# avianphysics/avian

Hardware: NVIDIA H100
Metric: physics steps/sec on 100k-cube stack (broad phase + solver stage per step) (higher is better)
Workload: dtype f32

## Files before the change

avian_b200/csrc/contact_rows.hpp:

```cpp
#pragma once
#include <cstdint>

#include "narrow_math.hpp"

namespace avn {

template <class S>
struct EdgeRows {
    int E;
    uint32_t* c1; uint32_t* c2; uint32_t* b1; uint32_t* b2; uint8_t* live;
    uint8_t* count; uint8_t* disjoint; S* normal; S* a1; S* a2; S* pen; S* ns;
    uint8_t* prev_count; double* prev_a1; double* prev_a2;
    S* ws_n_in; S* ws_t_in; S* ws_n_out; S* ws_t_out; S* nimp_in; S* nimp_out;
};

template <class S>
struct NarrowEdgeArgs {
    EdgeRows<S> r;
    const uint8_t* shape; const S* dims; const S* pos; const S* rot; const S* lv; const S* av; const S* amin; const S* amax;
    double dt, tol, thr2;
    int match;
};

template <class S> NM_HD inline nm::V3 ldd3(const S* p, size_t i) { return {double(p[3 * i]), double(p[3 * i + 1]), double(p[3 * i + 2])}; }
template <class S> NM_HD inline void std3(S* p, size_t i, nm::V3 v) { p[3 * i] = S(v.x); p[3 * i + 1] = S(v.y); p[3 * i + 2] = S(v.z); }

template <class S>
NM_HD inline void narrow_edge_row(const NarrowEdgeArgs<S>& a, int e) {
    const EdgeRows<S>& r = a.r;
    if (!r.live[e]) { r.count[e] = 0; r.disjoint[e] = 0; return; }
    const uint32_t ca = r.c1[e], cb = r.c2[e], ba = r.b1[e], bb = r.b2[e];
    int np = 0;
    nm::V3 normal{0, 0, 0};
    nm::PointOut out[4];
    bool disjoint = false;
    {
        const nm::V3 mina = ldd3(a.amin, ca), maxa = ldd3(a.amax, ca), minb = ldd3(a.amin, cb), maxb = ldd3(a.amax, cb);
        disjoint = (mina.x > maxb.x || maxa.x < minb.x || mina.y > maxb.y || maxa.y < minb.y || mina.z > maxb.z || maxa.z < minb.z);
    }
    r.disjoint[e] = disjoint ? 1 : 0;
    if (!disjoint) {
        const nm::V3 pa = ldd3(a.pos, ca), pb = ldd3(a.pos, cb);
        const nm::Q qa{double(a.rot[4 * size_t(ca)]), double(a.rot[4 * size_t(ca) + 1]), double(a.rot[4 * size_t(ca) + 2]), double(a.rot[4 * size_t(ca) + 3])};
        const nm::Q qb{double(a.rot[4 * size_t(cb)]), double(a.rot[4 * size_t(cb) + 1]), double(a.rot[4 * size_t(cb) + 2]), double(a.rot[4 * size_t(cb) + 3])};
        const nm::V3 v1 = ldd3(a.lv, ba), v2 = ldd3(a.lv, bb), w1 = ldd3(a.av, ba), w2 = ldd3(a.av, bb);
        const nm::V3 rel = v2 - v1;
        const double eff_margin = a.dt * nm::len(rel);
        const double max_dist = nm::smax(eff_margin, a.tol);
        nm::Contacts pts;
        const int ta = a.shape ? a.shape[ca] : nm::SHAPE_CUBOID, tb = a.shape ? a.shape[cb] : nm::SHAPE_CUBOID;
        if (nm::collide(ta, ldd3(a.dims, ca), pa, qa, tb, ldd3(a.dims, cb), pb, qb, max_dist, normal, pts))
            np = nm::manifold_points(pts, normal, pa, pb, rel, w1, w2, a.dt, eff_margin, out);
        else
            normal = nm::V3{0, 0, 0};
    }
    const int oc = r.prev_count[e];
    nm::V3 oa1[4], oa2[4];
    S on[4], otx[4], oty[4];
    for (int k = 0; k < oc; ++k) {
        const size_t q = size_t(e) * 4 + k;
        oa1[k] = nm::V3{r.prev_a1[3 * q], r.prev_a1[3 * q + 1], r.prev_a1[3 * q + 2]};
        oa2[k] = nm::V3{r.prev_a2[3 * q], r.prev_a2[3 * q + 1], r.prev_a2[3 * q + 2]};
        on[k] = r.ws_n_out[q]; otx[k] = r.ws_t_out[2 * q]; oty[k] = r.ws_t_out[2 * q + 1];
    }
    r.count[e] = uint8_t(np);
    std3(r.normal, size_t(e), normal);
    for (int k = 0; k < 4; ++k) {
        const size_t q = size_t(e) * 4 + k;
        S vn = S(0), vx = S(0), vy = S(0);
        if (k < np) {
            const int j = a.match ? nm::match_point(out[k].anchor1, out[k].anchor2, oa1, oa2, oc, a.thr2) : -1;
            if (j >= 0) { vn = on[j]; vx = otx[j]; vy = oty[j]; }
            std3(r.a1, q, out[k].anchor1);
            std3(r.a2, q, out[k].anchor2);
            r.pen[q] = S(out[k].penetration);
            r.ns[q] = S(out[k].normal_speed);
            r.prev_a1[3 * q] = out[k].anchor1.x; r.prev_a1[3 * q + 1] = out[k].anchor1.y; r.prev_a1[3 * q + 2] = out[k].anchor1.z;
            r.prev_a2[3 * q] = out[k].anchor2.x; r.prev_a2[3 * q + 1] = out[k].anchor2.y; r.prev_a2[3 * q + 2] = out[k].anchor2.z;
        } else {
            std3(r.a1, q, nm::V3{0, 0, 0});
            std3(r.a2, q, nm::V3{0, 0, 0});
            r.pen[q] = S(0);
            r.ns[q] = S(0);
        }
        r.ws_n_in[q] = vn;
        r.ws_t_in[2 * q] = vx;
        r.ws_t_in[2 * q + 1] = vy;
        r.ws_n_out[q] = vn;
        r.ws_t_out[2 * q] = vx;
        r.ws_t_out[2 * q + 1] = vy;
    }
    r.prev_count[e] = uint8_t(np);
}


}
```

avian_b200/csrc/contacts.cu:

```cuda
#include <cooperative_groups.h>

#include <algorithm>
#include <cstdlib>
#include <cstring>

#include "context.hpp"
#include "contact_rows.hpp"
#include "device_prims.cuh"

namespace avn {
namespace {
namespace cg = cooperative_groups;

enum { CH_NONE = 0, CH_PUSH = 1, CH_POP = 2, CH_REMOVE = 3, CH_MASK = 3, CH_DONE = 0x10 };
enum { ISL_NONE = 0, ISL_ADD = 1, ISL_REMOVE = 2 };

struct GraphCounters {
    uint32_t removed, started, stopped, changed, rounds, ovf_dirty, manifolds, any_restitution, aborted, bad_pairs;
    uint32_t round_left[3];
    uint32_t color_offsets[AVN_GRAPH_COLOR_COUNT + 1];
    uint32_t ovf_count;
};

struct GraphRows {
// ... 268 lines not shown
}

__global__ void pair_set_kernel(GraphRows g, uint64_t* __restrict__ table, uint64_t mask) {
    const int e = blockIdx.x * blockDim.x + threadIdx.x;
    if (e >= g.hw || !g.live[e]) return;
    const uint32_t a = g.c1[e], b = g.c2[e];
    const uint64_t k = (a < b ? (uint64_t(a) << 32) | b : (uint64_t(b) << 32) | a) + 1;
    uint64_t h = hash64(k) & mask;
    for (;;) {
        unsigned long long prev = atomicCAS((unsigned long long*)&table[h], 0ull, (unsigned long long)k);
        if (prev == 0ull || prev == k) return;
        h = (h + 1) & mask;
    }
}

__global__ void edge_add_kernel(int n, const uint32_t* __restrict__ ids, const uint32_t* __restrict__ c1, const uint32_t* __restrict__ c2,
                                const uint32_t* __restrict__ b1, const uint32_t* __restrict__ b2, uint32_t* rc1, uint32_t* rc2, uint32_t* rb1, uint32_t* rb2,
                                uint8_t* live, uint8_t* count, uint8_t* prev_count) {
    int k = blockIdx.x * blockDim.x + threadIdx.x;
    if (k >= n) return;
    const uint32_t e = ids[k];
    rc1[e] = c1[k]; rc2[e] = c2[k]; rb1[e] = b1[k]; rb2[e] = b2[k];
    live[e] = 1;
    count[e] = 0;
    prev_count[e] = 0;
}
__global__ void edge_remove_kernel(int n, const uint32_t* __restrict__ ids, uint8_t* live, uint8_t* count, uint8_t* prev_count) {
    int k = blockIdx.x * blockDim.x + threadIdx.x;
    if (k >= n) return;
    const uint32_t e = ids[k];
    live[e] = 0; count[e] = 0; prev_count[e] = 0;
}

template <class S>
__global__ void __launch_bounds__(128) narrow_edges_kernel(const __grid_constant__ NarrowEdgeArgs<S> a, uint8_t* fresh, int only_fresh) {
    const int e = blockIdx.x * blockDim.x + threadIdx.x;
    if (e >= a.r.E) return;
    if (only_fresh) {
        if (!fresh[e]) return;
        fresh[e] = 0;
    }
    narrow_edge_row<S>(a, e);
}


struct IslandCounters { uint32_t islands, sleeping, put_to_sleep, woken, split_bodies, merges, split_root, _pad; unsigned long long cand; };
constexpr uint32_t ISL_NONE_BODY = 0xffffffffu;

struct IslandState {
    int B;
    const uint8_t* kind;
    uint32_t* parent; uint32_t* root; uint32_t* root_prev; uint32_t* removed;
    uint8_t* isl_sleeping; uint8_t* awake; uint8_t* need_wake; uint8_t* touched; uint8_t* in_split;
    float* timer;
    const float* thr_lin; const float* thr_ang; const uint8_t* disabled; const uint8_t* host_wake;
    uint32_t* cand_body;
    IslandCounters* ctr;
    float time_to_sleep, delta_secs;
};
__device__ __forceinline__ bool isl_static(const IslandState& s, uint32_t b) { return b >= uint32_t(s.B) || s.kind[b] == AVN_BODY_STATIC; }
__device__ __forceinline__ uint32_t isl_find(uint32_t* parent, uint32_t x) {
    uint32_t p = *reinterpret_cast<volatile uint32_t*>(&parent[x]);
    while (p != x) {
        const uint32_t gp = *reinterpret_cast<volatile uint32_t*>(&parent[p]);
        if (gp != p) parent[x] = gp;
        x = p; p = gp;
    }
    return x;
}
__device__ __forceinline__ bool isl_union(uint32_t* parent, uint32_t u, uint32_t v) {
    for (;;) {
        uint32_t ru = isl_find(parent, u), rv = isl_find(parent, v);
        if (ru == rv) return false;
        if (ru < rv) { const uint32_t t = ru; ru = rv; rv = t; }
        if (atomicCAS(&parent[ru], ru, rv) == ru) return true;
// ... 120 lines not shown
    if (b >= s.B || isl_static(s, uint32_t(b)) || s.root[b] != uint32_t(b)) return;
    atomicAdd(&s.ctr->islands, 1u);
    if (!s.awake[b] && !s.isl_sleeping[b] && s.removed[b] == 0) { s.isl_sleeping[b] = 1; atomicAdd(&s.ctr->put_to_sleep, 1u); }
    if (s.isl_sleeping[b]) atomicAdd(&s.ctr->sleeping, 1u);
}
__global__ void isl_finish_kernel(IslandState s, uint32_t* __restrict__ out_island, uint8_t* __restrict__ out_sleeping) {
    const int b = blockIdx.x * blockDim.x + threadIdx.x;
    if (b >= s.B) return;
    const bool st = isl_static(s, uint32_t(b));
    const uint32_t r = st ? ISL_NONE_BODY : s.root[b];
    out_island[b] = r;
    out_sleeping[b] = (!st && s.isl_sleeping[r]) ? 1 : 0;
    s.root_prev[b] = st ? uint32_t(b) : r;
    s.awake[b] = 0; s.need_wake[b] = 0; s.touched[b] = 0; s.in_split[b] = 0;
    if (b == 0) {
        const unsigned long long c = s.ctr->cand;
        if (c != 0ull) *s.cand_body = 0xffffffffu - uint32_t(c & 0xffffffffull);
    }
}

template <class S>
class Contacts final : public ContactsBase {
   public:
    Contacts(cudaStream_t stream, ErrorSink* err) : stream_(stream), err_(err) {
        int dev = 0;
        cudaGetDevice(&dev);
        cudaDeviceProp prop;
        if (cudaGetDeviceProperties(&prop, dev) == cudaSuccess) sm_count_ = prop.multiProcessorCount;
        cudaHostAlloc(&h_ctr_, sizeof(GraphCounters), cudaHostAllocDefault);
        up_stream_ = stream_;
        if (cudaStreamCreateWithFlags(&copy_stream_, cudaStreamNonBlocking) != cudaSuccess) { (void)cudaGetLastError(); copy_stream_ = nullptr; }
        cudaEventCreateWithFlags(&ev_in_, cudaEventDisableTiming);
        if (const char* c = getenv("AVN_GRAPH_CLUSTER")) use_cluster_ = atoi(c) != 0;
    }
    ~Contacts() override {
        if (h_ctr_) cudaFreeHost(h_ctr_);
        if (h_isl_) cudaFreeHost(h_isl_);
        if (ev_in_) cudaEventDestroy(ev_in_);
        if (copy_stream_) { cudaStreamSynchronize(copy_stream_); cudaStreamDestroy(copy_stream_); }
    }

    AvnStatus reserve(uint32_t capacity) override {
        if (capacity <= E_) return AVN_OK;
        const size_t n = capacity;
        struct Col { DevBuf* buf; size_t bytes_per_row; };
        Col cols[] = {{&c1_, 4}, {&c2_, 4}, {&b1_, 4}, {&b2_, 4}, {&live_, 1}, {&count_, 1}, {&disjoint_, 1}, {&normal_, 3 * sizeof(S)}, {&a1_, 12 * sizeof(S)},
                      {&a2_, 12 * sizeof(S)}, {&pen_, 4 * sizeof(S)}, {&ns_, 4 * sizeof(S)}, {&prev_count_, 1}, {&prev_a1_, 12 * sizeof(double)},
                      {&prev_a2_, 12 * sizeof(double)}, {&ws_n_in_, 4 * sizeof(S)}, {&ws_t_in_, 8 * sizeof(S)}, {&ws_n_out_, 4 * sizeof(S)},
                      {&ws_t_out_, 8 * sizeof(S)}, {&nimp_in_, 4 * sizeof(S)}, {&nimp_out_, 4 * sizeof(S)},
                      {&pflags_, 1}, {&touching_, 1}, {&colour_, 1}, {&change_, 1}, {&old_colour_, 1}, {&ovf_pos_, 4}, {&ovf_, 4}, {&isl_event_, 1}, {&fresh_, 1}};
        for (Col& c : cols) {
            void* fresh = nullptr;
            AVN_CUDA(cudaMalloc(&fresh, n * c.bytes_per_row));
            AVN_CUDA(cudaMemsetAsync(fresh, 0, n * c.bytes_per_row, stream_));
            if (c.buf->p && E_) AVN_CUDA(cudaMemcpyAsync(fresh, c.buf->p, size_t(E_) * c.bytes_per_row, cudaMemcpyDeviceToDevice, stream_));
            AVN_CUDA(cudaStreamSynchronize(stream_));
            if (c.buf->p) cudaFree(c.buf->p);
            c.buf->p = fresh;
            c.buf->cap = n * c.bytes_per_row;
        }
        E_ = capacity;
        const size_t nblocks = (n + RS_TILE - 1) / RS_TILE;
        AVN_CUDA(k0_.ensure(n * 4)); AVN_CUDA(k1_.ensure(n * 4)); AVN_CUDA(v0_.ensure(n * 4)); AVN_CUDA(v1_.ensure(n * 4)); AVN_CUDA(list_.ensure(n * 4));
        AVN_CUDA(hist_.ensure(256 * nblocks * 4));
        AVN_CUDA(m_b1_.ensure(n * 4)); AVN_CUDA(m_b2_.ensure(n * 4)); AVN_CUDA(m_fr_.ensure(n * sizeof(S))); AVN_CUDA(m_re_.ensure(n * sizeof(S)));
        uint64_t cap = 1024;
// ... 357 lines not shown
        UPC(i_lv_, in->linear_velocity, 3 * B, S, in_.lv);
        UPC(i_av_, in->angular_velocity, 3 * B, S, in_.av);
        UPC(i_amin_, in->aabb_min, 3 * C, S, in_.amin);
        UPC(i_amax_, in->aabb_max, 3 * C, S, in_.amax);
#undef UPC
        up_stream_ = stream_;
        in_.colliders = C;
        return AVN_OK;
    }
    AvnStatus launch_narrow(const AvnNarrowParams* prm, const AvnNarrowInput* in, uint32_t match_contacts, double length_unit, uint32_t n) {
        bool only_fresh = false;
        if (prefetched_ == in) {
            AVN_CUDA(cudaStreamWaitEvent(stream_, ev_in_, 0));
            only_fresh = early_rows_ > 0;
            if (only_fresh && n == early_rows_ && !added_this_step_) { prefetched_ = nullptr; early_rows_ = 0; return AVN_OK; }
        } else {
            if (prefetched_) AVN_CUDA(cudaStreamWaitEvent(stream_, ev_in_, 0));
            AvnStatus st = upload_inputs(in, false, stream_);
            if (st != AVN_OK) return st;
        }
        prefetched_ = nullptr;
        early_rows_ = 0;
        return enqueue_narrow(prm, match_contacts, length_unit, n, stream_, only_fresh);
    }
    AvnStatus enqueue_narrow(const AvnNarrowParams* prm, uint32_t match_contacts, double length_unit, uint32_t n, cudaStream_t s, bool only_fresh) {
        NarrowEdgeArgs<S> a{};
        a.r = rows();
        a.r.E = int(n);
        a.shape = in_.shape; a.dims = in_.dims; a.pos = in_.pos; a.rot = in_.rot; a.lv = in_.lv; a.av = in_.av; a.amin = in_.amin; a.amax = in_.amax;
        a.dt = prm->dt;
        a.tol = prm->contact_tolerance;
        a.thr2 = (0.1 * length_unit) * (0.1 * length_unit);
        a.match = match_contacts ? 1 : 0;
        narrow_edges_kernel<S><<<(n + 127) / 128, 128, 0, s>>>(a, fresh_.as<uint8_t>(), only_fresh ? 1 : 0);
        AVN_CUDA(cudaGetLastError());
        return AVN_OK;
    }
    void radix_pass(int n) {
        const int nblocks = (n + RS_TILE - 1) / RS_TILE;
        rs_histogram<uint32_t><<<nblocks, RS_THREADS, 0, stream_>>>(k0_.as<uint32_t>(), n, 0, hist_.as<uint32_t>(), nblocks);
        if (nblocks <= RS_FUSE_MAX_BLOCKS) {
            rs_scatter<uint32_t, true><<<nblocks, RS_THREADS, 0, stream_>>>(k0_.as<uint32_t>(), v0_.as<uint32_t>(), n, 0, hist_.as<uint32_t>(), nblocks, k1_.as<uint32_t>(),
                                                                            v1_.as<uint32_t>());
        } else {
            rs_scan<<<1, 1024, 0, stream_>>>(hist_.as<uint32_t>(), 256 * nblocks);
            rs_scatter<uint32_t, false><<<nblocks, RS_THREADS, 0, stream_>>>(k0_.as<uint32_t>(), v0_.as<uint32_t>(), n, 0, hist_.as<uint32_t>(), nblocks, k1_.as<uint32_t>(),
                                                                             v1_.as<uint32_t>());
        }
    }
    GraphRows graph_rows() {
        GraphRows g{};
        g.hw = int(hw_);
        g.c1 = c1_.as<uint32_t>(); g.c2 = c2_.as<uint32_t>(); g.b1 = b1_.as<uint32_t>(); g.b2 = b2_.as<uint32_t>();
        g.live = live_.as<uint8_t>(); g.count = count_.as<uint8_t>(); g.disjoint = disjoint_.as<uint8_t>(); g.prev_count = prev_count_.as<uint8_t>();
        g.pflags = pflags_.as<uint8_t>(); g.touching = touching_.as<uint8_t>(); g.colour = colour_.as<uint8_t>(); g.change = change_.as<uint8_t>();
        g.old_colour = old_colour_.as<uint8_t>(); g.ovf_pos = ovf_pos_.as<uint32_t>(); g.ovf = ovf_.as<uint32_t>(); g.isl_event = isl_event_.as<uint8_t>(); g.fresh = fresh_.as<uint8_t>();
        g.body_kind = kind_.as<uint8_t>(); g.n_bodies = int(n_bodies_);
        g.body_bits = body_bits_.as<uint32_t>(); g.body_min = body_min_.as<unsigned long long>();
        g.ctr = ctr_.as<GraphCounters>();
        return g;
    }
    EdgeRows<S> rows() {
        EdgeRows<S> r{};
        r.E = int(E_);
        r.c1 = c1_.as<uint32_t>(); r.c2 = c2_.as<uint32_t>(); r.b1 = b1_.as<uint32_t>(); r.b2 = b2_.as<uint32_t>(); r.live = live_.as<uint8_t>();
        r.count = count_.as<uint8_t>(); r.disjoint = disjoint_.as<uint8_t>(); r.normal = normal_.as<S>(); r.a1 = a1_.as<S>(); r.a2 = a2_.as<S>();
        r.pen = pen_.as<S>(); r.ns = ns_.as<S>(); r.prev_count = prev_count_.as<uint8_t>(); r.prev_a1 = prev_a1_.as<double>(); r.prev_a2 = prev_a2_.as<double>();
// ... 52 lines not shown
```

avian_b200/csrc/narrow_math.hpp:

```cpp
#pragma once
#include <cmath>

#if defined(__CUDACC__)
#define NM_HD __host__ __device__
#define NM_COLD __host__ __device__ __noinline__
#define NM_ROLLED _Pragma("unroll 1")
#else
#define NM_HD
#define NM_COLD
#define NM_ROLLED
#endif

namespace nm {

using S = double;

struct V3 { S x, y, z; };
NM_HD inline V3 operator+(V3 a, V3 b) { return {a.x + b.x, a.y + b.y, a.z + b.z}; }
NM_HD inline V3 operator-(V3 a, V3 b) { return {a.x - b.x, a.y - b.y, a.z - b.z}; }
NM_HD inline V3 operator-(V3 a) { return {-a.x, -a.y, -a.z}; }
NM_HD inline V3 operator*(V3 a, S s) { return {a.x * s, a.y * s, a.z * s}; }
NM_HD inline S dot(V3 a, V3 b) { return a.x * b.x + a.y * b.y + a.z * b.z; }
NM_HD inline V3 cross(V3 a, V3 b) { return {a.y * b.z - a.z * b.y, a.z * b.x - a.x * b.z, a.x * b.y - a.y * b.x}; }
NM_HD inline S len(V3 a) { return sqrt(dot(a, a)); }
NM_HD inline S comp(V3 a, int i) { return i == 0 ? a.x : (i == 1 ? a.y : a.z); }
NM_HD inline S smax(S a, S b) { return a < b ? b : a; }
NM_HD inline S smin(S a, S b) { return b < a ? b : a; }

struct Q { S x, y, z, w; };
NM_HD inline V3 rot(Q q, V3 v) {
    V3 b{q.x, q.y, q.z};
    S b2 = dot(b, b);
    return v * (q.w * q.w - b2) + b * (dot(v, b) * 2) + cross(b, v) * (q.w * 2);
}
struct M3 { V3 c[3]; };
NM_HD inline M3 to_mat(Q q) { return {{rot(q, {1, 0, 0}), rot(q, {0, 1, 0}), rot(q, {0, 0, 1})}}; }

enum ShapeType { SHAPE_CUBOID = 0, SHAPE_SPHERE = 1 };
struct Box { V3 c; M3 r; V3 he; };

constexpr int MAX_RAW_POINTS = 8;
struct Witness { V3 a, b; };
struct Contacts {
    int n;
    Witness p[MAX_RAW_POINTS];
    NM_HD void clear() { n = 0; }
    NM_HD void push(V3 on_a, V3 on_b) { p[n].a = on_a; p[n].b = on_b; ++n; }
};

NM_HD inline void box_face(const Box& b, int axis, S sign, V3 out[4]) {
    int u = (axis + 1) % 3, v = (axis + 2) % 3;
    V3 n = b.r.c[axis] * (sign * comp(b.he, axis));
    V3 eu = b.r.c[u] * comp(b.he, u), ev = b.r.c[v] * comp(b.he, v);
    V3 fc = b.c + n;
    out[0] = fc + eu + ev; out[1] = fc - eu + ev; out[2] = fc - eu - ev; out[3] = fc + eu - ev;
}

NM_HD inline int clip_poly(const V3* in, int n, V3 plane_n, S plane_d, V3* out) {
    int m = 0;
    for (int i = 0; i < n; ++i) {
        V3 a = in[i], b = in[(i + 1) % n];
        S da = dot(plane_n, a) - plane_d, db = dot(plane_n, b) - plane_d;
        if (da <= 0) out[m++] = a;
        if ((da < 0 && db > 0) || (da > 0 && db < 0)) out[m++] = a + (b - a) * (da / (da - db));
    }
    return m;
}

NM_HD inline S box_radius(const Box& b, V3 n) {
    return fabs(dot(b.r.c[0], n)) * b.he.x + fabs(dot(b.r.c[1], n)) * b.he.y + fabs(dot(b.r.c[2], n)) * b.he.z;
}

NM_HD inline bool segment_closest(V3 p, V3 u, S hu, V3 q, V3 w, S hw, S& s, S& t) {
    V3 r = p - q;
    S a = dot(u, u), e = dot(w, w), f = dot(w, r), c = dot(u, r), b = dot(u, w);
    S den = a * e - b * b;
    S s0 = den > 1e-12 ? (b * f - c * e) / den : 0;
    s = smax(-hu, smin(hu, s0));
    bool end = den <= 1e-12 || s != s0;
    t = (b * s + f) / e;
    if (t < -hw || t > hw) {
        t = t < -hw ? -hw : hw;
        s = smax(-hu, smin(hu, (b * t - c) / a));
        end = true;
    }
    return end;
}

NM_HD inline S box_point_closest(const Box& b, V3 p, V3& on) {
    V3 d = p - b.c;
    on = b.c;
    for (int k = 0; k < 3; ++k) on = on + b.r.c[k] * smax(-comp(b.he, k), smin(comp(b.he, k), dot(d, b.r.c[k])));
    V3 e = p - on;
    return dot(e, e);
}

NM_COLD inline S box_box_closest(const Box& A, const Box& B, V3& on_a, V3& on_b) {
    S best = 1e300;
NM_ROLLED
    for (int side = 0; side < 2; ++side) {
        const Box& P = side == 0 ? A : B;
        const Box& O = side == 0 ? B : A;
NM_ROLLED
        for (int m = 0; m < 8; ++m) {
            V3 v = P.c + P.r.c[0] * (m & 1 ? P.he.x : -P.he.x) + P.r.c[1] * (m & 2 ? P.he.y : -P.he.y) + P.r.c[2] * (m & 4 ? P.he.z : -P.he.z);
            V3 on;
            S d2 = box_point_closest(O, v, on);
            if (d2 < best) { best = d2; on_a = side == 0 ? v : on; on_b = side == 0 ? on : v; }
        }
    }
    auto edge_mid = [](const Box& b, int k, int m) {
        int u = (k + 1) % 3, v = (k + 2) % 3;
        return b.c + b.r.c[u] * (m & 1 ? comp(b.he, u) : -comp(b.he, u)) + b.r.c[v] * (m & 2 ? comp(b.he, v) : -comp(b.he, v));
    };
NM_ROLLED
    for (int ei = 0; ei < 12; ++ei) {
        const int i = ei >> 2, mi = ei & 3;
        V3 pa = edge_mid(A, i, mi);
NM_ROLLED
        for (int ej = 0; ej < 12; ++ej) {
            const int j = ej >> 2, mj = ej & 3;
            V3 pb = edge_mid(B, j, mj);
            S s, t;
            segment_closest(pa, A.r.c[i], comp(A.he, i), pb, B.r.c[j], comp(B.he, j), s, t);
            V3 qa = pa + A.r.c[i] * s, qb = pb + B.r.c[j] * t, e = qb - qa;
            S d2 = dot(e, e);
            if (d2 < best) { best = d2; on_a = qa; on_b = qb; }
        }
    }
    return sqrt(best);
}

NM_HD inline bool closest_pair(V3 on_a, V3 on_b, S dist, S max_dist, V3& normal, Contacts& pts) {
    pts.clear();
    if (dist > max_dist) return false;
    if (dist > 1e-12) normal = (on_b - on_a) * (1 / dist);
    pts.push(on_a, on_b);
    return true;
}

constexpr S FACE_GAP_SLACK = 1e-4;

NM_HD inline bool box_box(const Box& A, const Box& B, S max_dist, V3& normal, Contacts& pts) {
    pts.clear();
    V3 d = B.c - A.c;
    S best_sep = -1e300;
    int best_kind = -1, best_i = 0, best_j = 0;
    V3 best_n{0, 1, 0};
    auto consider = [&](V3 n, int kind, int i, int j, S bias) {
        S l = len(n);
        if (l < 1e-9) return;
        n = n * (1 / l);
        if (dot(n, d) < 0) n = -n;
        S sep = dot(n, d) - box_radius(A, n) - box_radius(B, n);
        if (sep - bias > best_sep + 1e-9) { best_sep = sep - bias; best_kind = kind; best_i = i; best_j = j; best_n = n; }
    };
    for (int i = 0; i < 3; ++i) consider(A.r.c[i], 0, i, 0, 0);
    for (int i = 0; i < 3; ++i) consider(B.r.c[i], 1, i, 0, 0);
    const S face_sep = best_sep;
    const int face_kind = best_kind, face_i = best_i;
    const V3 face_n = best_n;
    for (int i = 0; i < 3; ++i)
        for (int j = 0; j < 3; ++j) consider(cross(A.r.c[i], B.r.c[j]), 2, i, j, 1e-4);
    S sep = best_kind == 2 ? best_sep + 1e-4 : best_sep;
    if (sep > max_dist) return false;
    normal = best_n;
    if (best_kind == 2) {
        V3 ea = A.r.c[best_i], eb = B.r.c[best_j];
        V3 pa = A.c, pb = B.c;
        for (int k = 0; k < 3; ++k) {
            if (k != best_i) pa = pa + A.r.c[k] * (comp(A.he, k) * (dot(A.r.c[k], normal) > 0 ? 1 : -1));
            if (k != best_j) pb = pb + B.r.c[k] * (comp(B.he, k) * (dot(B.r.c[k], normal) < 0 ? 1 : -1));
        }
        S s, t;
        if (!segment_closest(pa, ea, comp(A.he, best_i), pb, eb, comp(B.he, best_j), s, t)) {
            pts.push(pa + ea * s, pb + eb * t);
            return true;
        }
        if (sep > 0) {
            V3 on_a, on_b;
            S dist = box_box_closest(A, B, on_a, on_b);
            return closest_pair(on_a, on_b, dist, max_dist, normal, pts);
        }
        sep = face_sep; best_kind = face_kind; best_i = face_i; normal = face_n;
    }
    const bool ref_is_a = best_kind == 0;
    const Box& R = ref_is_a ? A : B;
    const Box& I = ref_is_a ? B : A;
    V3 rn = ref_is_a ? normal : -normal;
    int inc_axis = 0;
    S inc_best = -1;
    for (int k = 0; k < 3; ++k) {
        S v = fabs(dot(I.r.c[k], rn));
        if (v > inc_best) { inc_best = v; inc_axis = k; }
    }
    S isign = dot(I.r.c[inc_axis], rn) > 0 ? -1 : 1;
    V3 poly[16], tmp[16];
    box_face(I, inc_axis, isign, poly);
    int np = 4;
    int u = (best_i + 1) % 3, v = (best_i + 2) % 3;
    const int axes[2] = {u, v};
    for (int a = 0; a < 2 && np > 0; ++a) {
        V3 sn = R.r.c[axes[a]];
        S he = comp(R.he, axes[a]);
        np = clip_poly(poly, np, sn, dot(sn, R.c) + he, tmp);
        np = clip_poly(tmp, np, -sn, -dot(sn, R.c) + he, poly);
    }
    S face_d = dot(rn, R.c) + comp(R.he, best_i) * 1.0;
    S nearest = 1e300;
    for (int k = 0; k < np; ++k) {
        S dist = dot(rn, poly[k]) - face_d;
        if (dist > max_dist) continue;
        nearest = smin(nearest, dist);
        V3 on_ref = poly[k] - rn * dist;
        bool dup = false;
        for (int q = 0; q < pts.n; ++q) {
            V3 e = (ref_is_a ? pts.p[q].b : pts.p[q].a) - poly[k];
            if (dot(e, e) < 1e-12) { dup = true; break; }
        }
        if (dup) continue;
        if (pts.n == MAX_RAW_POINTS) break;
        if (ref_is_a) pts.push(on_ref, poly[k]); else pts.push(poly[k], on_ref);
    }
    if (sep > 0 && nearest > sep + FACE_GAP_SLACK) {
        V3 on_a, on_b;
        S dist = box_box_closest(A, B, on_a, on_b);
        if (nearest > dist + FACE_GAP_SLACK) return closest_pair(on_a, on_b, dist, max_dist, normal, pts);
    }
    return pts.n != 0;
}

NM_HD inline void prune4(Contacts& pts, V3 n) {
    if (pts.n <= 4) return;
    auto depth = [&](int i) { return dot(pts.p[i].a - pts.p[i].b, n); };
    int p0 = 0;
    for (int i = 1; i < pts.n; ++i) if (depth(i) > depth(p0) + 1e-12) p0 = i;
    int p1 = p0;
    S best = -1;
    for (int i = 0; i < pts.n; ++i) { V3 e = pts.p[i].a - pts.p[p0].a; S v = dot(e, e); if (v > best) { best = v; p1 = i; } }
    V3 dir = cross(pts.p[p1].a - pts.p[p0].a, n);
    int p2 = p0, p3 = p0;
    S mx = 0, mn = 0;
    for (int i = 0; i < pts.n; ++i) {
        S v = dot(pts.p[i].a - pts.p[p0].a, dir);
        if (v > mx) { mx = v; p2 = i; }
        if (v < mn) { mn = v; p3 = i; }
    }
    bool keep[MAX_RAW_POINTS] = {false, false, false, false, false, false, false, false};
    keep[p0] = keep[p1] = keep[p2] = keep[p3] = true;
    int m = 0;
    for (int i = 0; i < pts.n; ++i)
        if (keep[i]) pts.p[m++] = pts.p[i];
    pts.n = m;
}

NM_HD inline bool sphere_sphere(V3 ca, S ra, V3 cb, S rb, S max_dist, V3& normal, Contacts& pts) {
    pts.clear();
    V3 d = cb - ca;
    S l = len(d);
    if (l - ra - rb > max_dist) return false;
    normal = l > 1e-12 ? d * (1 / l) : V3{0, 1, 0};
    pts.push(ca + normal * ra, cb - normal * rb);
    return true;
}

NM_HD inline bool box_sphere(const Box& A, V3 cs, S rs, S max_dist, V3& normal, Contacts& pts) {
    pts.clear();
    V3 d = cs - A.c;
    V3 local{dot(d, A.r.c[0]), dot(d, A.r.c[1]), dot(d, A.r.c[2])};
    V3 cl{smax(-A.he.x, smin(A.he.x, local.x)), smax(-A.he.y, smin(A.he.y, local.y)), smax(-A.he.z, smin(A.he.z, local.z))};
    V3 on_box = A.c + A.r.c[0] * cl.x + A.r.c[1] * cl.y + A.r.c[2] * cl.z;
    V3 e = cs - on_box;
    S l = len(e);
    const bool inside = fabs(local.x) <= A.he.x && fabs(local.y) <= A.he.y && fabs(local.z) <= A.he.z;
    if (!inside && l > 1e-9) {
        if (l - rs > max_dist) return false;
        normal = e * (1 / l);
    } else {
        int ax = 0; S best = 1e300;
        for (int k = 0; k < 3; ++k) { S v = comp(A.he, k) - fabs(comp(local, k)); if (v < best) { best = v; ax = k; } }
        S sgn = comp(local, ax) >= 0 ? 1 : -1;
        normal = A.r.c[ax] * sgn;
        on_box = cs + normal * best;
    }
    pts.push(on_box, cs - normal * rs);
    return true;
}

NM_HD inline bool collide(int type_a, V3 he_a, V3 pa, Q qa, int type_b, V3 he_b, V3 pb, Q qb, S max_dist, V3& normal, Contacts& pts) {
    pb = pb - pa;
    pa = V3{0, 0, 0};
    bool hit;
    if (type_a == SHAPE_CUBOID && type_b == SHAPE_CUBOID) {
        Box A{pa, to_mat(qa), he_a}, B{pb, to_mat(qb), he_b};
        hit = box_box(A, B, max_dist, normal, pts);
        if (hit) prune4(pts, normal);
    } else if (type_a == SHAPE_SPHERE && type_b == SHAPE_SPHERE) {
        hit = sphere_sphere(pa, he_a.x, pb, he_b.x, max_dist, normal, pts);
    } else if (type_a == SHAPE_CUBOID) {
        Box A{pa, to_mat(qa), he_a};
        hit = box_sphere(A, pb, he_b.x, max_dist, normal, pts);
    } else {
        Box B{pb, to_mat(qb), he_b};
        hit = box_sphere(B, pa, he_a.x, max_dist, normal, pts);
        if (hit) {
            normal = -normal;
            for (int k = 0; k < pts.n; ++k) { V3 t = pts.p[k].a; pts.p[k].a = pts.p[k].b; pts.p[k].b = t; }
        }
    }
    return hit;
}

struct PointOut { V3 anchor1, anchor2; S penetration, normal_speed; };

NM_HD inline int manifold_points(const Contacts& pts, V3 normal, V3 pa, V3 pb, V3 rel, V3 w1, V3 w2, S dt, S eff_margin, PointOut out[4]) {
    int m = 0;
    for (int k = 0; k < pts.n && m < 4; ++k) {
        PointOut pt;
        pt.anchor1 = pts.p[k].a;
        pt.anchor2 = pts.p[k].b - (pb - pa);
        pt.penetration = dot(pts.p[k].a - pts.p[k].b, normal);
        V3 rv = rel + cross(w2, pt.anchor2) - cross(w1, pt.anchor1);
        pt.normal_speed = dot(rv, normal);
        bool keep = -pt.penetration < eff_margin || (pt.normal_speed * dt - pt.penetration < eff_margin);
        if (!keep) continue;
        out[m++] = pt;
    }
    return m;
}

NM_HD inline int match_point(V3 anchor1, V3 anchor2, const V3* old_anchor1, const V3* old_anchor2, int n_old, S thr2) {
    for (int k = 0; k < n_old; ++k) {
        V3 e11 = anchor1 - old_anchor1[k], e22 = anchor2 - old_anchor2[k], e12 = anchor1 - old_anchor2[k], e21 = anchor2 - old_anchor1[k];
        if ((dot(e11, e11) < thr2 && dot(e22, e22) < thr2) || (dot(e12, e12) < thr2 && dot(e21, e21) < thr2)) return k;
    }
    return -1;
}

}
```

avian_b200/csrc/solver_host.cu:

```cuda
#include <algorithm>
#include <cmath>
#include <cstdlib>
#include <cstring>

#include "context.hpp"
#include "joint_schedule.hpp"
#include "solver_kernels.cuh"

namespace avn {

namespace {

template <class S>
Soft<S> softness(S damping_ratio, S hz, S delta_secs) {
    S double_damping_ratio = S(2) * damping_ratio;
    S angular_frequency = S(6.283185307179586476925286766559) * hz;
    S a1 = double_damping_ratio + angular_frequency * delta_secs;
    S a2 = angular_frequency * delta_secs * a1;
    S a3 = S(1) / (S(1) + a2);
    Soft<S> s;
    s.bias = angular_frequency / a1;
    s.mass_scale = a2 * a3;
    s.impulse_scale = a3;
    return s;
}

template <class S>
class Solver final : public SolverBase {
   public:
    Solver(cudaStream_t stream, ErrorSink* err, uint32_t cfg_flags, int device) : stream_(stream), err_(err), cfg_flags_(cfg_flags) {
        cudaDeviceProp prop;
        if (cudaGetDeviceProperties(&prop, device) == cudaSuccess) {
            sm_count_ = prop.multiProcessorCount;
            coop_ok_ = prop.cooperativeLaunch != 0;
        }
        {
            const char* lp = getenv("AVN_L2_PERSIST");
            l2_persist_ = !(lp && !strcmp(lp, "0")) && prop.persistingL2CacheMaxSize > 0;
            if (l2_persist_) {
                l2_persist_bytes_ = std::min<size_t>(size_t(prop.persistingL2CacheMaxSize), size_t(64) << 20);
                l2_window_max_ = size_t(prop.accessPolicyMaxWindowSize);
                if (cudaDeviceSetLimit(cudaLimitPersistingL2CacheSize, l2_persist_bytes_) != cudaSuccess) { (void)cudaGetLastError(); l2_persist_ = false; }
            }
        }
        const char* mode = getenv("AVN_LAUNCH_MODE");
        if (mode && !strcmp(mode, "phases")) use_mega_ = false;
        if (mode && !strcmp(mode, "barrier")) use_wave_ = false;
        const char* bps = getenv("AVN_MEGA_BPS");
        mega_bps_ = bps ? atoi(bps) : (sizeof(S) == 8 ? 2 : 3);
        if (mega_bps_ < 2 || mega_bps_ > 4) mega_bps_ = 3;
        if (mode && !strcmp(mode, "wave")) force_wave_ = true;
        coop_ok_ = coop_ok_ && select_megakernel(AVN_MAX_MANIFOLD_POINTS);
        for (auto& e : ev_) cudaEventCreate(&e);
        up_stream_ = stream_;
        if (cudaStreamCreateWithFlags(&copy_stream_, cudaStreamNonBlocking) != cudaSuccess) { (void)cudaGetLastError(); copy_stream_ = nullptr; }
        cudaEventCreateWithFlags(&ev_prefetch_, cudaEventDisableTiming);
    }
    ~Solver() override {
        for (auto& e : ev_) cudaEventDestroy(e);
        if (ev_prefetch_) cudaEventDestroy(ev_prefetch_);
        if (copy_stream_) { cudaStreamSynchronize(copy_stream_); cudaStreamDestroy(copy_stream_); }
        if (h_agree_) cudaFreeHost(h_agree_);
    }

    AvnStatus upload(const AvnStepParams* prm, AvnBodyColumns* bc, AvnManifoldColumns* mc, AvnJointSet* js) override;
    AvnStatus upload_edges(const AvnStepParams* prm, AvnBodyColumns* bc, AvnEdgeManifolds* em, AvnJointSet* js) override;
    AvnStatus upload_graph(const AvnStepParams* prm, AvnBodyColumns* bc, const AvnEdgeManifolds* graph, ContactsBase* contacts, AvnJointSet* js) override;
    AvnStatus upload_resident(const AvnStepParams* prm, AvnBodyColumns* bc, ContactsBase* contacts, AvnJointSet* js) override;
    AvnStatus run_range(uint32_t first, uint32_t count, uint32_t flags) override;
    AvnStatus set_boundary(const AvnBoundary* bnd) override;
    AvnStatus boundary_snapshot() override;
    AvnStatus boundary_pack(void* device_table) override;
    AvnStatus boundary_apply(const void* device_gathered) override;
    AvnStatus step_partitioned(CommBase* comm) override;
    int needs_restitution() const override { return host_any_restitution_ ? 1 : 0; }
    AvnStatus prefetch_bodies(AvnBodyColumns* bc, uint32_t flags) override {
        if (!bc) return err_->fail(AVN_ERR_INVALID_ARGUMENT, "bodies are required");
        if (bc->count && (!bc->position || !bc->rotation || !bc->linear_velocity || !bc->angular_velocity || !bc->inverse_mass || !bc->inverse_inertia_local))
            return err_->fail(AVN_ERR_INVALID_ARGUMENT, "bodies: position, rotation, velocities, inverse_mass and inverse_inertia_local are required");
        prefetched_ = false;
        if (!copy_stream_) return AVN_OK;
// ... 69 lines not shown
        UPS(b_ma_, bc.max_angular_speed, B, S, max_ang);
#undef UPS
#undef UPB
        bcols_.kind = d.kind; bcols_.locked = d.locked; bcols_.dominance = d.dominance; bcols_.integ_flags = d.integ_flags;
        bcols_.position = d.position; bcols_.rotation = d.rotation; bcols_.linvel = d.linvel; bcols_.angvel = d.angvel; bcols_.inv_mass = d.inv_mass;
        bcols_.inv_inertia_local = d.inv_inertia_local; bcols_.com = d.com; bcols_.lin_damp = d.lin_damp; bcols_.ang_damp = d.ang_damp;
        bcols_.grav_scale = d.grav_scale; bcols_.lin_acc = d.lin_acc; bcols_.ang_acc = d.ang_acc; bcols_.max_lin = d.max_lin; bcols_.max_ang = d.max_ang;
        bcols_.count = B;
        return AVN_OK;
    }
    AvnStatus build_joint_schedule(const AvnBodyColumns& bc, const AvnJointSet& js);
    template <int OP> void launch_phase(int begin, int count, bool serial = false) {
        if (count <= 0) return;
        int grid = serial ? 1 : std::min((count + kBlock - 1) / kBlock, sm_count_ * 8);
        const bool contact_op = OP == OP_WARM || OP == OP_SOLVE_BIAS || OP == OP_RELAX || OP == OP_RESTITUTION;
        const size_t smem = contact_op ? stage_bytes<S>(kBlock) : 0;
        if (smem > 48 * 1024) cudaFuncSetAttribute(phase_kernel<S, OP>, cudaFuncAttributeMaxDynamicSharedMemorySize, int(smem));
        phase_kernel<S, OP><<<grid, kBlock, smem, stream_>>>(dev_, begin, count, serial ? 1 : 0);
        ++launches_;
    }
    template <int OP> void launch_contact_pass() {
        const int* off = dev_.color_off;
        launch_phase<OP>(off[AVN_COLOR_OVERFLOW], dev_.color_len[AVN_COLOR_OVERFLOW], true);
        for (int c = 0; c < AVN_COLOR_OVERFLOW; ++c) launch_phase<OP>(off[c], dev_.color_len[c]);
    }

    cudaStream_t stream_;
    ErrorSink* err_;
    uint32_t cfg_flags_;
    int sm_count_ = 132;
    bool coop_ok_ = false, use_mega_ = true, use_wave_ = true, l2_persist_ = false;
    size_t l2_persist_bytes_ = 0, l2_window_max_ = 0;
    int mega_grid_ = 0, mega_bps_ = 3, mega_maxp_ = 0, mega_sel_bps_ = 0;
    bool force_wave_ = false;

    template <int MAXP> const void* mega_variant(int bps) const {
        switch (bps) {
            case 2: return (const void*)step_megakernel<S, 2, MAXP>;
            case 4: return (const void*)step_megakernel<S, 4, MAXP>;
            default: return (const void*)step_megakernel<S, 3, MAXP>;
        }
    }
    static size_t mega_smem_bytes(int maxp) { return stage_bytes<S>(MEGA_BLOCK, maxp); }
    bool select_megakernel(int max_points, int bps = 0) {
        const int maxp = max_points <= 1 ? 1 : AVN_MAX_MANIFOLD_POINTS;
        if (bps == 0) bps = mega_bps_;
        if (maxp == mega_maxp_ && bps == mega_sel_bps_) return mega_grid_ > 0;
        mega_maxp_ = maxp;
        mega_sel_bps_ = bps;
        mega_fn_ = maxp == 1 ? mega_variant<1>(bps) : mega_variant<AVN_MAX_MANIFOLD_POINTS>(bps);
        const size_t smem = mega_smem_bytes(maxp);
        int per_sm = 0;
        mega_grid_ = 0;
        if (cudaFuncSetAttribute(mega_fn_, cudaFuncAttributeMaxDynamicSharedMemorySize, int(smem)) == cudaSuccess &&
            cudaOccupancyMaxActiveBlocksPerMultiprocessor(&per_sm, mega_fn_, MEGA_BLOCK, smem) == cudaSuccess && per_sm > 0)
            mega_grid_ = per_sm * sm_count_;
        else
            (void)cudaGetLastError();
        if (getenv("AVN_DEBUG_GRID")) fprintf(stderr, "[avn] megakernel bps=%d maxp=%d: %d blocks/SM resident, grid %d, %zu B dynamic smem\n", bps, maxp, per_sm, mega_grid_, smem);
        return mega_grid_ > 0;
    }
    int max_np_ = AVN_MAX_MANIFOLD_POINTS;
    const void* mega_fn_ = nullptr;
    cudaEvent_t ev_[EV_COUNT];
    AvnTimings tm_{};
    uint32_t launches_ = 0, exchanges_ = 0;
    size_t h2d_bytes_ = 0;
// ... 392 lines not shown
            hj_ = *js;
        }
    }
#undef UP
    cudaEventRecord(ev_[EV_H2D1], stream_);
    uploaded_ = true;
    prepared_ = false;
    ran_ = false;
    dev_.bnd_of = nullptr;
    dev_.vel_ref = nullptr;
    bnd_n_ = 0;
    bnd_slots_ = 0;
    tm_ = AvnTimings{};
    return AVN_OK;
}

template <class S>
AvnStatus Solver<S>::run() {
    return run_range(0, dev_.substeps, AVN_RUN_PREPARE | AVN_RUN_RESTITUTION | AVN_RUN_FINALIZE);
}

template <class S>
AvnStatus Solver<S>::run_range(uint32_t first, uint32_t count, uint32_t flags) {
    if (!uploaded_) return err_->fail(AVN_ERR_INVALID_ARGUMENT, "avn_solver_run before avn_solver_upload");
    const bool prepare = (flags & AVN_RUN_PREPARE) != 0;
    if (!prepare && !prepared_) return err_->fail(AVN_ERR_INVALID_ARGUMENT, "avn_solver_run_range: the first launch after an upload must include AVN_RUN_PREPARE");
    if (uint64_t(first) + count > uint64_t(dev_.substeps)) return err_->fail(AVN_ERR_INVALID_ARGUMENT, "avn_solver_run_range: substeps [%u, %u) exceed %d", first, first + count, dev_.substeps);
    dev_.do_prepare = prepare ? 1 : 0;
    dev_.sub_begin = int(first);
    dev_.sub_end = int(first + count);
    dev_.do_restitution = (flags & AVN_RUN_RESTITUTION) ? 1 : 0;
    dev_.do_finalize = (flags & AVN_RUN_FINALIZE) ? 1 : 0;
    bool mega = use_mega_ && coop_ok_;
    if (prepare) step_bps_ = mega_bps_;
    mega = mega && select_megakernel(max_np_, step_bps_);
    if (prepare) {
        launches_ = 0;
        cudaEventRecord(ev_[EV_RUN0], stream_);
        AVN_CUDA(cudaMemsetAsync(dev_.any_restitution, 0, FLAG_WORDS * sizeof(int) + 8 * sizeof(unsigned long long), stream_));
        int widest_colour = 0;
        for (int c = 0; c < AVN_COLOR_OVERFLOW; ++c) widest_colour = std::max(widest_colour, dev_.color_len[c]);
        const bool chain_bound = force_wave_ || widest_colour <= 2 * mega_grid_ * MEGA_BLOCK;
        dev_.wave = (mega && use_wave_ && chain_bound && dev_.M > 0 && dev_.J == 0 && dev_.color_len[AVN_COLOR_OVERFLOW] == 0) ? 1 : 0;
        if (dev_.M > 0) {
            AVN_CUDA(cudaMemsetAsync(dev_.cst + size_t(CP_IDX) * dev_.Mpad, 0, size_t(dev_.Mpad) * sizeof(Vec4<S>), stream_));
        }
        if (dev_.wave) {
            AVN_CUDA(cudaMemsetAsync(dev_.ver, 0, (size_t(dev_.B) + 1) * sizeof(unsigned), stream_));
            AVN_CUDA(cudaMemsetAsync(dev_.deg, 0, 2 * (size_t(dev_.B) + 1) * sizeof(int), stream_));
        }
        mega_step_ = mega;
    } else {
        mega = mega && mega_step_;
    }
    if (l2_persist_ && hot_bytes_ > 0) {
        cudaStreamAttrValue attr{};
        attr.accessPolicyWindow.base_ptr = hot_.p;
        attr.accessPolicyWindow.num_bytes = std::min(hot_bytes_, l2_window_max_);
        attr.accessPolicyWindow.hitRatio = float(std::min(1.0, double(l2_persist_bytes_) / double(attr.accessPolicyWindow.num_bytes)));
        attr.accessPolicyWindow.hitProp = cudaAccessPropertyPersisting;
        attr.accessPolicyWindow.missProp = cudaAccessPropertyStreaming;
        cudaStreamSetAttribute(stream_, cudaStreamAttributeAccessPolicyWindow, &attr);
    }
    const DevSolver<S>& d = dev_;
    if (mega) {
        void* args[] = {(void*)&dev_};
        cudaError_t e = cudaLaunchCooperativeKernel(mega_fn_, dim3(mega_grid_), dim3(MEGA_BLOCK), args, mega_smem_bytes(mega_maxp_), stream_);
        if (e != cudaSuccess) {
            (void)cudaGetLastError();
            if (!prepare && dev_.wave)
                return err_->fail(AVN_ERR_CUDA, "cooperative launch refused in the middle of a wavefront-scheduled step: %s", cudaGetErrorString(e));
            mega = false;
            mega_step_ = false;
            dev_.wave = 0;
// ... 299 lines not shown
```

Baseline: 428.3.

## Move narrow-phase scratch arrays to shared memory and widen solver blocks for wide colours

The narrow-phase kernel now keeps its per-thread clip polygons, witness points, manifold outputs and old-impulse arrays in a dynamic shared-memory slice instead of local-memory stack arrays. The slice stride is odd in 8-byte words to avoid bank conflicts, and the kernel requests two blocks per SM. The goal is to remove local-memory spills in the box-box clipping path, at the cost of a large shared-memory footprint per block that may cap occupancy. Separately, the f32 solver megakernel now picks 4 blocks per SM when the widest colour is large and no joints exist, unless AVN_MEGA_BPS is set.

Result: faster. 445.6 (median of 6 runs) (+4.0%).

```diff
diff --git a/avian_b200/csrc/contact_rows.hpp b/avian_b200/csrc/contact_rows.hpp
--- a/avian_b200/csrc/contact_rows.hpp
+++ b/avian_b200/csrc/contact_rows.hpp
@@ -26,13 +26,22 @@
 template <class S> NM_HD inline void std3(S* p, size_t i, nm::V3 v) { p[3 * i] = S(v.x); p[3 * i + 1] = S(v.y); p[3 * i + 2] = S(v.z); }
 
 template <class S>
-NM_HD inline void narrow_edge_row(const NarrowEdgeArgs<S>& a, int e) {
+struct RowArrays {
+    nm::V3 poly[nm::MAX_CLIP_POINTS], tmp[nm::MAX_CLIP_POINTS];
+    nm::Witness pts[nm::MAX_RAW_POINTS];
+    nm::PointOut out[4];
+    nm::V3 oa1[4], oa2[4];
+    S on[4], otx[4], oty[4];
+};
+
+template <class S, class Scratch>
+NM_HD inline void narrow_edge_row(const NarrowEdgeArgs<S>& a, int e, Scratch& sc) {
     const EdgeRows<S>& r = a.r;
     if (!r.live[e]) { r.count[e] = 0; r.disjoint[e] = 0; return; }
     const uint32_t ca = r.c1[e], cb = r.c2[e], ba = r.b1[e], bb = r.b2[e];
     int np = 0;
     nm::V3 normal{0, 0, 0};
-    nm::PointOut out[4];
+    auto out = sc.out;
     bool disjoint = false;
     {
         const nm::V3 mina = ldd3(a.amin, ca), maxa = ldd3(a.amax, ca), minb = ldd3(a.amin, cb), maxb = ldd3(a.amax, cb);
@@ -47,16 +56,16 @@
         const nm::V3 rel = v2 - v1;
         const double eff_margin = a.dt * nm::len(rel);
         const double max_dist = nm::smax(eff_margin, a.tol);
-        nm::Contacts pts;
+        nm::ContactsIn<nm::Witness*> pts{0, sc.pts};
         const int ta = a.shape ? a.shape[ca] : nm::SHAPE_CUBOID, tb = a.shape ? a.shape[cb] : nm::SHAPE_CUBOID;
-        if (nm::collide(ta, ldd3(a.dims, ca), pa, qa, tb, ldd3(a.dims, cb), pb, qb, max_dist, normal, pts))
+        if (nm::collide(ta, ldd3(a.dims, ca), pa, qa, tb, ldd3(a.dims, cb), pb, qb, max_dist, normal, pts, sc.poly, sc.tmp))
             np = nm::manifold_points(pts, normal, pa, pb, rel, w1, w2, a.dt, eff_margin, out);
         else
             normal = nm::V3{0, 0, 0};
     }
     const int oc = r.prev_count[e];
-    nm::V3 oa1[4], oa2[4];
-    S on[4], otx[4], oty[4];
+    auto oa1 = sc.oa1, oa2 = sc.oa2;
+    auto on = sc.on, otx = sc.otx, oty = sc.oty;
     for (int k = 0; k < oc; ++k) {
         const size_t q = size_t(e) * 4 + k;
         oa1[k] = nm::V3{r.prev_a1[3 * q], r.prev_a1[3 * q + 1], r.prev_a1[3 * q + 2]};
@@ -92,6 +101,11 @@
     }
     r.prev_count[e] = uint8_t(np);
 }
+template <class S>
+inline void narrow_edge_row(const NarrowEdgeArgs<S>& a, int e) {
+    RowArrays<S> sc;
+    narrow_edge_row(a, e, sc);
+}
 
 
 }
diff --git a/avian_b200/csrc/contacts.cu b/avian_b200/csrc/contacts.cu
--- a/avian_b200/csrc/contacts.cu
+++ b/avian_b200/csrc/contacts.cu
@@ -324,15 +324,38 @@
     live[e] = 0; count[e] = 0; prev_count[e] = 0;
 }
 
+constexpr int NARROW_THREADS = 128;
+constexpr int NARROW_REGION_P = nm::MAX_CLIP_POINTS * int(sizeof(nm::V3));
+constexpr int NARROW_REGION_T = nm::MAX_RAW_POINTS * int(sizeof(nm::Witness));
+constexpr int NARROW_SLICE = NARROW_REGION_P + NARROW_REGION_T + 8;
+static_assert(NARROW_REGION_P >= 4 * int(sizeof(nm::PointOut)) && NARROW_REGION_T >= nm::MAX_CLIP_POINTS * int(sizeof(nm::V3)) &&
+              NARROW_REGION_T >= 8 * int(sizeof(nm::V3)) + 12 * 8 && (NARROW_SLICE / 8) % 2 == 1, "narrow scratch layout");
+constexpr int NARROW_SMEM = NARROW_THREADS * NARROW_SLICE;
+
+struct RowScratch {
+    nm::V3* poly; nm::V3* tmp;
+    nm::Witness* pts;
+    nm::PointOut* out;
+    nm::V3* oa1; nm::V3* oa2;
+    double* on; double* otx; double* oty;
+};
+
 template <class S>
-__global__ void __launch_bounds__(128) narrow_edges_kernel(const __grid_constant__ NarrowEdgeArgs<S> a, uint8_t* fresh, int only_fresh) {
-    const int e = blockIdx.x * blockDim.x + threadIdx.x;
+__global__ void __launch_bounds__(NARROW_THREADS, 2) narrow_edges_kernel(const __grid_constant__ NarrowEdgeArgs<S> a, uint8_t* fresh, int only_fresh) {
+    extern __shared__ __align__(16) char narrow_smem[];
+    const int t = threadIdx.x, e = blockIdx.x * NARROW_THREADS + t;
     if (e >= a.r.E) return;
     if (only_fresh) {
         if (!fresh[e]) return;
         fresh[e] = 0;
     }
-    narrow_edge_row<S>(a, e);
+    char* const rp = narrow_smem + t * NARROW_SLICE;
+    char* const rt = rp + NARROW_REGION_P;
+    nm::V3* const old = reinterpret_cast<nm::V3*>(rt);
+    double* const imp = reinterpret_cast<double*>(old + 8);
+    RowScratch sc{reinterpret_cast<nm::V3*>(rp), reinterpret_cast<nm::V3*>(rt), reinterpret_cast<nm::Witness*>(rt),
+                  reinterpret_cast<nm::PointOut*>(rp), old, old + 4, imp, imp + 4, imp + 8};
+    narrow_edge_row<S>(a, e, sc);
 }
 
 
@@ -519,6 +542,7 @@
         if (cudaStreamCreateWithFlags(&copy_stream_, cudaStreamNonBlocking) != cudaSuccess) { (void)cudaGetLastError(); copy_stream_ = nullptr; }
         cudaEventCreateWithFlags(&ev_in_, cudaEventDisableTiming);
         if (const char* c = getenv("AVN_GRAPH_CLUSTER")) use_cluster_ = atoi(c) != 0;
+        cudaFuncSetAttribute(narrow_edges_kernel<S>, cudaFuncAttributeMaxDynamicSharedMemorySize, NARROW_SMEM);
     }
     ~Contacts() override {
         if (h_ctr_) cudaFreeHost(h_ctr_);
@@ -942,7 +966,7 @@
         a.tol = prm->contact_tolerance;
         a.thr2 = (0.1 * length_unit) * (0.1 * length_unit);
         a.match = match_contacts ? 1 : 0;
-        narrow_edges_kernel<S><<<(n + 127) / 128, 128, 0, s>>>(a, fresh_.as<uint8_t>(), only_fresh ? 1 : 0);
+        narrow_edges_kernel<S><<<(n + NARROW_THREADS - 1) / NARROW_THREADS, NARROW_THREADS, NARROW_SMEM, s>>>(a, fresh_.as<uint8_t>(), only_fresh ? 1 : 0);
         AVN_CUDA(cudaGetLastError());
         return AVN_OK;
     }
diff --git a/avian_b200/csrc/narrow_math.hpp b/avian_b200/csrc/narrow_math.hpp
--- a/avian_b200/csrc/narrow_math.hpp
+++ b/avian_b200/csrc/narrow_math.hpp
@@ -34,24 +34,29 @@
     return v * (q.w * q.w - b2) + b * (dot(v, b) * 2) + cross(b, v) * (q.w * 2);
 }
 struct M3 { V3 c[3]; };
+NM_HD inline V3 col(const M3& m, int i) { return i == 0 ? m.c[0] : (i == 1 ? m.c[1] : m.c[2]); }
 NM_HD inline M3 to_mat(Q q) { return {{rot(q, {1, 0, 0}), rot(q, {0, 1, 0}), rot(q, {0, 0, 1})}}; }
 
 enum ShapeType { SHAPE_CUBOID = 0, SHAPE_SPHERE = 1 };
 struct Box { V3 c; M3 r; V3 he; };
 
 constexpr int MAX_RAW_POINTS = 8;
+constexpr int MAX_CLIP_POINTS = 16;
 struct Witness { V3 a, b; };
-struct Contacts {
+
+template <class W>
+struct ContactsIn {
     int n;
-    Witness p[MAX_RAW_POINTS];
+    W p;
     NM_HD void clear() { n = 0; }
     NM_HD void push(V3 on_a, V3 on_b) { p[n].a = on_a; p[n].b = on_b; ++n; }
 };
+using Contacts = ContactsIn<Witness[MAX_RAW_POINTS]>;
 
 NM_HD inline void box_face(const Box& b, int axis, S sign, V3 out[4]) {
     int u = (axis + 1) % 3, v = (axis + 2) % 3;
-    V3 n = b.r.c[axis] * (sign * comp(b.he, axis));
-    V3 eu = b.r.c[u] * comp(b.he, u), ev = b.r.c[v] * comp(b.he, v);
+    V3 n = col(b.r, axis) * (sign * comp(b.he, axis));
+    V3 eu = col(b.r, u) * comp(b.he, u), ev = col(b.r, v) * comp(b.he, v);
     V3 fc = b.c + n;
     out[0] = fc + eu + ev; out[1] = fc - eu + ev; out[2] = fc - eu - ev; out[3] = fc + eu - ev;
 }
@@ -95,7 +100,7 @@
     return dot(e, e);
 }
 
-NM_COLD inline S box_box_closest(const Box& A, const Box& B, V3& on_a, V3& on_b) {
+NM_COLD inline S box_box_closest(Box A, Box B, V3& on_a, V3& on_b) {
     S best = 1e300;
 NM_ROLLED
     for (int side = 0; side < 2; ++side) {
@@ -131,7 +136,8 @@
     return sqrt(best);
 }
 
-NM_HD inline bool closest_pair(V3 on_a, V3 on_b, S dist, S max_dist, V3& normal, Contacts& pts) {
+template <class C>
+NM_HD inline bool closest_pair(V3 on_a, V3 on_b, S dist, S max_dist, V3& normal, C& pts) {
     pts.clear();
     if (dist > max_dist) return false;
     if (dist > 1e-12) normal = (on_b - on_a) * (1 / dist);
@@ -141,7 +147,8 @@
 
 constexpr S FACE_GAP_SLACK = 1e-4;
 
-NM_HD inline bool box_box(const Box& A, const Box& B, S max_dist, V3& normal, Contacts& pts) {
+template <class C>
+NM_HD inline bool box_box(const Box& A, const Box& B, S max_dist, V3& normal, C& pts, V3* poly, V3* tmp) {
     pts.clear();
     V3 d = B.c - A.c;
     S best_sep = -1e300;
@@ -166,7 +173,7 @@
     if (sep > max_dist) return false;
     normal = best_n;
     if (best_kind == 2) {
-        V3 ea = A.r.c[best_i], eb = B.r.c[best_j];
+        V3 ea = col(A.r, best_i), eb = col(B.r, best_j);
         V3 pa = A.c, pb = B.c;
         for (int k = 0; k < 3; ++k) {
             if (k != best_i) pa = pa + A.r.c[k] * (comp(A.he, k) * (dot(A.r.c[k], normal) > 0 ? 1 : -1));
@@ -185,8 +192,8 @@
         sep = face_sep; best_kind = face_kind; best_i = face_i; normal = face_n;
     }
     const bool ref_is_a = best_kind == 0;
-    const Box& R = ref_is_a ? A : B;
-    const Box& I = ref_is_a ? B : A;
+    const Box R = ref_is_a ? A : B;
+    const Box I = ref_is_a ? B : A;
     V3 rn = ref_is_a ? normal : -normal;
     int inc_axis = 0;
     S inc_best = -1;
@@ -194,14 +201,13 @@
         S v = fabs(dot(I.r.c[k], rn));
         if (v > inc_best) { inc_best = v; inc_axis = k; }
     }
-    S isign = dot(I.r.c[inc_axis], rn) > 0 ? -1 : 1;
-    V3 poly[16], tmp[16];
+    S isign = dot(col(I.r, inc_axis), rn) > 0 ? -1 : 1;
     box_face(I, inc_axis, isign, poly);
     int np = 4;
     int u = (best_i + 1) % 3, v = (best_i + 2) % 3;
     const int axes[2] = {u, v};
     for (int a = 0; a < 2 && np > 0; ++a) {
-        V3 sn = R.r.c[axes[a]];
+        V3 sn = col(R.r, axes[a]);
         S he = comp(R.he, axes[a]);
         np = clip_poly(poly, np, sn, dot(sn, R.c) + he, tmp);
         np = clip_poly(tmp, np, -sn, -dot(sn, R.c) + he, poly);
@@ -230,7 +236,8 @@
     return pts.n != 0;
 }
 
-NM_HD inline void prune4(Contacts& pts, V3 n) {
+template <class C>
+NM_HD inline void prune4(C& pts, V3 n) {
     if (pts.n <= 4) return;
     auto depth = [&](int i) { return dot(pts.p[i].a - pts.p[i].b, n); };
     int p0 = 0;
@@ -246,15 +253,15 @@
         if (v > mx) { mx = v; p2 = i; }
         if (v < mn) { mn = v; p3 = i; }
     }
-    bool keep[MAX_RAW_POINTS] = {false, false, false, false, false, false, false, false};
-    keep[p0] = keep[p1] = keep[p2] = keep[p3] = true;
+    const unsigned keep = 1u << p0 | 1u << p1 | 1u << p2 | 1u << p3;
     int m = 0;
     for (int i = 0; i < pts.n; ++i)
-        if (keep[i]) pts.p[m++] = pts.p[i];
+        if (keep >> i & 1u) pts.p[m++] = pts.p[i];
     pts.n = m;
 }
 
-NM_HD inline bool sphere_sphere(V3 ca, S ra, V3 cb, S rb, S max_dist, V3& normal, Contacts& pts) {
+template <class C>
+NM_HD inline bool sphere_sphere(V3 ca, S ra, V3 cb, S rb, S max_dist, V3& normal, C& pts) {
     pts.clear();
     V3 d = cb - ca;
     S l = len(d);
@@ -264,7 +271,8 @@
     return true;
 }
 
-NM_HD inline bool box_sphere(const Box& A, V3 cs, S rs, S max_dist, V3& normal, Contacts& pts) {
+template <class C>
+NM_HD inline bool box_sphere(const Box& A, V3 cs, S rs, S max_dist, V3& normal, C& pts) {
     pts.clear();
     V3 d = cs - A.c;
     V3 local{dot(d, A.r.c[0]), dot(d, A.r.c[1]), dot(d, A.r.c[2])};
@@ -280,20 +288,21 @@
         int ax = 0; S best = 1e300;
         for (int k = 0; k < 3; ++k) { S v = comp(A.he, k) - fabs(comp(local, k)); if (v < best) { best = v; ax = k; } }
         S sgn = comp(local, ax) >= 0 ? 1 : -1;
-        normal = A.r.c[ax] * sgn;
+        normal = col(A.r, ax) * sgn;
         on_box = cs + normal * best;
     }
     pts.push(on_box, cs - normal * rs);
     return true;
 }
 
-NM_HD inline bool collide(int type_a, V3 he_a, V3 pa, Q qa, int type_b, V3 he_b, V3 pb, Q qb, S max_dist, V3& normal, Contacts& pts) {
+template <class C>
+NM_HD inline bool collide(int type_a, V3 he_a, V3 pa, Q qa, int type_b, V3 he_b, V3 pb, Q qb, S max_dist, V3& normal, C& pts, V3* poly, V3* tmp) {
     pb = pb - pa;
     pa = V3{0, 0, 0};
     bool hit;
     if (type_a == SHAPE_CUBOID && type_b == SHAPE_CUBOID) {
         Box A{pa, to_mat(qa), he_a}, B{pb, to_mat(qb), he_b};
-        hit = box_box(A, B, max_dist, normal, pts);
+        hit = box_box(A, B, max_dist, normal, pts, poly, tmp);
         if (hit) prune4(pts, normal);
     } else if (type_a == SHAPE_SPHERE && type_b == SHAPE_SPHERE) {
         hit = sphere_sphere(pa, he_a.x, pb, he_b.x, max_dist, normal, pts);
@@ -310,10 +319,15 @@
     }
     return hit;
 }
+NM_HD inline bool collide(int type_a, V3 he_a, V3 pa, Q qa, int type_b, V3 he_b, V3 pb, Q qb, S max_dist, V3& normal, Contacts& pts) {
+    V3 poly[MAX_CLIP_POINTS], tmp[MAX_CLIP_POINTS];
+    return collide(type_a, he_a, pa, qa, type_b, he_b, pb, qb, max_dist, normal, pts, poly, tmp);
+}
 
 struct PointOut { V3 anchor1, anchor2; S penetration, normal_speed; };
 
-NM_HD inline int manifold_points(const Contacts& pts, V3 normal, V3 pa, V3 pb, V3 rel, V3 w1, V3 w2, S dt, S eff_margin, PointOut out[4]) {
+template <class C>
+NM_HD inline int manifold_points(const C& pts, V3 normal, V3 pa, V3 pb, V3 rel, V3 w1, V3 w2, S dt, S eff_margin, PointOut out[4]) {
     int m = 0;
     for (int k = 0; k < pts.n && m < 4; ++k) {
         PointOut pt;
diff --git a/avian_b200/csrc/solver_host.cu b/avian_b200/csrc/solver_host.cu
--- a/avian_b200/csrc/solver_host.cu
+++ b/avian_b200/csrc/solver_host.cu
@@ -47,6 +47,7 @@
         if (mode && !strcmp(mode, "phases")) use_mega_ = false;
         if (mode && !strcmp(mode, "barrier")) use_wave_ = false;
         const char* bps = getenv("AVN_MEGA_BPS");
+        bps_fixed_ = bps != nullptr;
         mega_bps_ = bps ? atoi(bps) : (sizeof(S) == 8 ? 2 : 3);
         if (mega_bps_ < 2 || mega_bps_ > 4) mega_bps_ = 3;
         if (mode && !strcmp(mode, "wave")) force_wave_ = true;
@@ -182,7 +183,7 @@
     bool coop_ok_ = false, use_mega_ = true, use_wave_ = true, l2_persist_ = false;
     size_t l2_persist_bytes_ = 0, l2_window_max_ = 0;
     int mega_grid_ = 0, mega_bps_ = 3, mega_maxp_ = 0, mega_sel_bps_ = 0;
-    bool force_wave_ = false;
+    bool force_wave_ = false, bps_fixed_ = false;
 
     template <int MAXP> const void* mega_variant(int bps) const {
         switch (bps) {
@@ -641,14 +642,17 @@
     dev_.do_restitution = (flags & AVN_RUN_RESTITUTION) ? 1 : 0;
     dev_.do_finalize = (flags & AVN_RUN_FINALIZE) ? 1 : 0;
     bool mega = use_mega_ && coop_ok_;
-    if (prepare) step_bps_ = mega_bps_;
+    int widest_colour = 0;
+    for (int c = 0; c < AVN_COLOR_OVERFLOW; ++c) widest_colour = std::max(widest_colour, dev_.color_len[c]);
+    if (prepare) {
+        const bool wide = sizeof(S) == 4 && dev_.J == 0 && 2 * widest_colour >= 3 * MEGA_BLOCK * sm_count_;
+        step_bps_ = wide && !bps_fixed_ ? 4 : mega_bps_;
+    }
     mega = mega && select_megakernel(max_np_, step_bps_);
     if (prepare) {
         launches_ = 0;
         cudaEventRecord(ev_[EV_RUN0], stream_);
         AVN_CUDA(cudaMemsetAsync(dev_.any_restitution, 0, FLAG_WORDS * sizeof(int) + 8 * sizeof(unsigned long long), stream_));
-        int widest_colour = 0;
-        for (int c = 0; c < AVN_COLOR_OVERFLOW; ++c) widest_colour = std::max(widest_colour, dev_.color_len[c]);
         const bool chain_bound = force_wave_ || widest_colour <= 2 * mega_grid_ * MEGA_BLOCK;
         dev_.wave = (mega && use_wave_ && chain_bound && dev_.M > 0 && dev_.J == 0 && dev_.color_len[AVN_COLOR_OVERFLOW] == 0) ? 1 : 0;
         if (dev_.M > 0) {
```
